# kogdenko/con-gen

Hardware: AMD Instinct MI355X
Metric: Gpkts/s + GB/s device-resident checksum, 64B & 1500B batches; %HBM peak (higher is better)
Workload: dtype u16; 1 GPU; 16777216 x 1500 B IPv4+TCP per GPU, dense stride 1500, ip_cksum + tcp_cksum per packet (BASELINE configs[2]; configs[4] at 8 GPUs); packets_per_gpu=16777216, packet_bytes=1500, parallelism=batch-split x1

## Files before the change

### con-gen_amd/csrc/cgck_dense_kernel.inc

```

constexpr int kDsS = 6;
constexpr uint32_t kDsSlot = kDsS * 1024;
constexpr int kDsChunks = kDsS * 64;
static_assert(((15 + 3 * 1520) >> 4) + 16 * (kDsS - 1) + 15 < kDsChunks, "a reducing lane's chunk lies in its slot");

template <int D, int C, bool W, int F>
__global__ __launch_bounds__(128) void CGCK_DSTR_KERNEL(KParams p)
{
	constexpr bool IP6 = CGCK_DSTR_IP6;
	static_assert(!IP6 || (W && F == 0), "the IPv6 variant is the product shape's: writer wave, no register frames");
	extern __shared__ __attribute__((aligned(16))) uint8_t smem[];
	const int lane = threadIdx.x & 63, g = lane >> 4, gl = lane & 15;
	const int wave = __builtin_amdgcn_readfirstlane(threadIdx.x >> 6);
	const uint32_t flags = p.flags;
	const bool raw = flags & CGCK_RAW;
	const int len = (int)p.ip_len;
	const uint32_t lds0 = __builtin_amdgcn_readfirstlane((uint32_t)(uintptr_t)smem);
	uint32_t *so = reinterpret_cast<uint32_t *>(smem + D * kDsSlot);
	const uint8_t *zero = (const uint8_t *)p.zero + (blockIdx.x & 63) * 64;
	const uint64_t base = reinterpret_cast<uint64_t>(p.base) + p.l3_off;
	const uint64_t n = p.n, stride = p.stride;
	constexpr uint32_t SC = 4 * C + F;
	const uint64_t NC = (n + SC - 1) / SC, G = gridDim.x, b = blockIdx.x;
	if (b >= NC)
		return;
	const uint32_t nsteps = (uint32_t)((NC - b + G - 1) / G * C);
	const uint32_t mode = p.contig;
	auto cfirst = [&](uint32_t k) { return (b + (uint64_t)k * G) * SC; };

	auto fin = [&](uint32_t tot, uint32_t ip, uint32_t ps, uint32_t hd, uint32_t proto) {
		const int hl = (int)hd * 4;
		uint32_t lo = 0, hi = 0;
		if (raw) {
			lo = finish(tot);
		} else if (len >= hl) {
			if (flags & CGCK_IP)
				lo = finish(ip);
			if (flags & CGCK_L4) {
				uint32_t L = ocsub(tot, ip);
				if (!(flags & CGCK_L4_NOPSEUDO))
					L = fold16(L + ps + (proto << 8) + bswap16((uint32_t)(len - hl) & 0xffffu));
				hi = finish(L);
			}
		}
		return lo | (hi << 16);
	};

	auto flush = [&](uint32_t k, const uint32_t *sb) {
		const uint64_t first = cfirst(k);
		if (first + 4 * C <= n) {
			if (lane < C) {
				const uint4 v4 = reinterpret_cast<const uint4 *>(sb)[lane];
				bstore16<kSc1>(out_rsrc(p.out + first, 16 * C), 16 * lane, u32x4_t{v4.x, v4.y, v4.z, v4.w});
			}
		} else {
			for (int i = lane; i < 4 * C; i += 64)
				if (first + i < n)
					gbl(p.out)[first + i] = sb[i];
		}
	};

	auto reg_frame = [&](uint64_t f, uint64_t a, int nch, const uint4 (&w)[kDsS]) __attribute__((always_inline)) {
		const int q = (int)(a & 15);
		uint32_t body = 0;
		uint4 tw = make_uint4(0, 0, 0, 0);
		bool ht = false;
#pragma unroll
		for (int s2 = 0; s2 < kDsS; ++s2) {
			const int c = 16 * s2 + gl;
			body += c < nch ? sum4(w[s2], 0u) : 0u;
			const bool t = c == nch - 1;
			const uint32_t mt = opaque(t ? ~0u : 0u);
			tw = make_uint4(pick(mt, w[s2].x, tw.x), pick(mt, w[s2].y, tw.y), pick(mt, w[s2].z, tw.z),
					pick(mt, w[s2].w, tw.w));
			ht = ht || t;
		}
		uint32_t corr = 0;
		if (gl == 0) {
			corr = hsum(q >= 4 ? w[0].x : 0u, 0);
			corr = hsum(q >= 8 ? w[0].y : 0u, corr);
			corr = hsum(q >= 12 ? w[0].z : 0u, corr);
		}
		if (ht) {
			const int e = q + len - 16 * (nch - 1);
			if ((len & 3) == 0) {
				corr = hsum(e <= 4 ? tw.y : 0u, corr);
				corr = hsum(e <= 8 ? tw.z : 0u, corr);
				corr = hsum(e <= 12 ? tw.w : 0u, corr);
			} else {
				corr = msum(tw, 0, e, 16, corr);
			}
		}
		uint32_t tot = fold16(body) + (0xffffu - fold16(corr));
		tot = fold16(gsum<16>(tot));
		const uint32_t n0 = __builtin_amdgcn_mov_dpp(w[0].x, 0x101, 0xF, 0xF, false);
		const uint32_t n1 = __builtin_amdgcn_mov_dpp(w[0].y, 0x101, 0xF, 0xF, false);
		const uint32_t n2 = __builtin_amdgcn_mov_dpp(w[0].z, 0x101, 0xF, 0xF, false);
		const uint32_t n3 = __builtin_amdgcn_mov_dpp(w[0].w, 0x101, 0xF, 0xF, false);
		const uint32_t d[8] = {w[0].x, w[0].y, w[0].z, w[0].w, n0, n1, n2, n3};
		const int q4 = q >> 2;
		const uint32_t m0 = opaque(q4 == 0 ? ~0u : 0u), m1 = opaque(q4 == 1 ? ~0u : 0u),
			       m2 = opaque(q4 == 2 ? ~0u : 0u);
		uint32_t h[5];
#pragma unroll
		for (int i = 0; i < 5; ++i)
			h[i] = pick(m0, d[i], pick(m1, d[i + 1], pick(m2, d[i + 2], d[i + 3])));
		const uint32_t hd = h[0] & 15;
		uint32_t ip = hsum(h[4], hsum(h[3], hsum(h[2], hsum(h[1], hsum(h[0], 0)))));
		if (gl == 0 && f < n) {
			if (hd != 5) {
				ip = 0;
				for (uint32_t i = 0; i < hd; ++i)
					ip = hsum(*gbl_at<const uint32_t>(a + 4 * i), ip);
			}
			const uint32_t r = fin(tot, fold16(ip), fold16(hsum(h[4], hsum(h[3], 0))), hd, (h[2] >> 8) & 0xffu);
			gbl(p.out)[f] = r;
			if (p.verdict)
				gbl(p.verdict)[f] = (uint8_t)(!raw && len < (int)hd * 4 ? CGCK_BAD_LEN : 0);
		}
	};

	if (W && wave == 1) {
		for (uint32_t j = 0; j < nsteps; ++j) {
			if (mode == 6)
				wg_barrier();
			if ((j + 1) % C == 0) {
				const uint32_t k = j / C;
				uint4 rw[F > 0 ? F / 4 : 1][kDsS];
				uint64_t ra[F > 0 ? F / 4 : 1];
				int rn[F > 0 ? F / 4 : 1];
#pragma unroll
				for (int u = 0; u < F / 4; ++u) {
					const uint64_t f = cfirst(k) + 4 * C + 4 * u + g;
					ra[u] = base + (f < n ? f : 0) * stride;
					rn[u] = f < n ? (int)(((ra[u] & 15) + len + 15) >> 4) : 0;
					const uint4 *c0 = reinterpret_cast<const uint4 *>(ra[u] & ~(uint64_t)15);
#pragma unroll
					for (int s2 = 0; s2 < kDsS; ++s2)
						rw[u][s2] = ldc<true>(c0, 16 * s2 + gl, rn[u], p.zero);
				}
				wg_barrier();
				const uint32_t *sb = so + (k & 1) * 8 * C;
				const uint64_t first = cfirst(k);
				for (int i = lane; i < 4 * C; i += 64) {
					const uint32_t v0 = sb[i], v1 = sb[4 * C + i];
					const uint32_t hd = (v1 >> 16) & 15u;
					if constexpr (IP6) {
						uint32_t bl = 0;
						const uint32_t r6 = first + i < n ? v6_dense(base + (first + i) * stride, len, v0 & 0xffffu,
											     v0 >> 16, v1 >> 24, flags, &bl)
										  : 0u;
						if (p.verdict && first + i < n)
							gbl(p.verdict)[first + i] = (uint8_t)bl;
						if (first + 4 * C <= n)
							bstore4<kSc1>(out_rsrc(p.out + first, 16 * C), 4 * i, r6);
						else if (first + i < n)
							gbl(p.out)[first + i] = r6;
						continue;
					}
					const uint32_t r = fin(v0 & 0xffffu, v0 >> 16, v1 & 0xffffu, hd, v1 >> 24);
					if (p.verdict && first + i < n)
						gbl(p.verdict)[first + i] = (uint8_t)(!raw && len < (int)hd * 4 ? CGCK_BAD_LEN : 0);
					if (first + 4 * C <= n)
						bstore4<kSc1>(out_rsrc(p.out + first, 16 * C), 4 * i, r);
					else if (first + i < n)
						gbl(p.out)[first + i] = r;
				}
#pragma unroll
				for (int u = 0; u < F / 4; ++u)
					reg_frame(cfirst(k) + 4 * C + 4 * u + g, ra[u], rn[u], rw[u]);
			}
		}
		return;
	}

	auto sfirst = [&](uint32_t j) { return cfirst(j / C) + 4 * (j % C); };
	auto issue = [&](uint32_t j) {
		const uint64_t f0 = sfirst(j);
		const bool live = j < nsteps && f0 < n;
		const uint64_t fl = f0 + 3 < n ? f0 + 3 : n - 1;
		const uint64_t a = (base + f0 * stride) & ~(uint64_t)15;
		const uint64_t e = (base + fl * stride + len - 1) & ~(uint64_t)15;
		const uint32_t slot = lds0 + (j % D) * kDsSlot;
#pragma unroll
		for (int i = 0; i < kDsS; ++i) {
			const uint64_t s0 = a + 1024 * i, src = s0 + 16 * lane;
			if (live && s0 + 1008 <= e)
				glds16_nt(reinterpret_cast<const void *>(src), slot + 1024 * i);
			else
				glds16_nt(live && src <= e ? reinterpret_cast<const void *>(src) : zero, slot + 1024 * i);
		}
	};
#pragma unroll
	for (int d = 0; d < D; ++d)
		issue(d);
	for (uint32_t j = 0; j < nsteps; ++j) {
		if (!W && j >= (uint32_t)C && (j % C) <= (uint32_t)(D - 1))
			asm volatile("s_waitcnt vmcnt(%0)" ::"i"(kDsS * (D - 1) + 1) : "memory");
		else
			asm volatile("s_waitcnt vmcnt(%0)" ::"i"(kDsS * (D - 1)) : "memory");
		if (!W || mode == 6)
			wg_barrier();
		uint32_t *sc = so + (W ? ((j / C) & 1) * 8 * C : 0);
		if (mode == 3) {
			issue(j + D);
		} else {
			const uint64_t f0 = sfirst(j);
			const uint64_t a = (base + f0 * stride) & ~(uint64_t)15;
			const int o = (int)(base + (f0 + g) * stride - a);
			const int q = o & 15, c0 = o >> 4;
			const int nch = (q + len + 15) >> 4;
			const uint8_t *sl = smem + (j % D) * kDsSlot;
			uint4 w[kDsS];
#pragma unroll
			for (int s = 0; s < kDsS; ++s) {
				const int c = c0 + 16 * s + gl;
				w[s] = *reinterpret_cast<const uint4 *>(sl + 16 * c);
			}
#if CGCK_DSTR_REGHDR
			asm volatile("s_waitcnt lgkmcnt(0)" ::: "memory");
			issue(j + D);
			uint4 wt = make_uint4(0, 0, 0, 0);
			bool ht = false;
#pragma unroll
			for (int s = 0; s < kDsS; ++s) {
				const bool t = 16 * s + gl == nch - 1;
				const uint32_t mt = opaque(t ? ~0u : 0u);
				wt = make_uint4(pick(mt, w[s].x, wt.x), pick(mt, w[s].y, wt.y), pick(mt, w[s].z, wt.z),
						pick(mt, w[s].w, wt.w));
				ht = ht || t;
			}
			const uint32_t n0 = __builtin_amdgcn_mov_dpp(w[0].x, 0x101, 0xF, 0xF, false);
			const uint32_t n1 = __builtin_amdgcn_mov_dpp(w[0].y, 0x101, 0xF, 0xF, false);
			const uint32_t n2 = __builtin_amdgcn_mov_dpp(w[0].z, 0x101, 0xF, 0xF, false);
			const uint32_t n3 = __builtin_amdgcn_mov_dpp(w[0].w, 0x101, 0xF, 0xF, false);
			const uint32_t dd[8] = {w[0].x, w[0].y, w[0].z, w[0].w, n0, n1, n2, n3};
			const int q4 = q >> 2;
			const uint32_t m0 = opaque(q4 == 0 ? ~0u : 0u), m1 = opaque(q4 == 1 ? ~0u : 0u),
				       m2 = opaque(q4 == 2 ? ~0u : 0u);
			uint32_t hh[5];
#pragma unroll
			for (int i = 0; i < 5; ++i)
				hh[i] = pick(m0, dd[i], pick(m1, dd[i + 1], pick(m2, dd[i + 2], dd[i + 3])));
			const uint32_t h1 = hh[1], h2 = hh[2], h3 = hh[3], h4 = hh[4];
			const uint32_t hd = hh[0] & 15;
			uint32_t ip = IP6 ? hsum(h1, hsum(hh[0], 0)) : hsum(h4, hsum(h3, hsum(h2, hsum(h1, hsum(hh[0], 0)))));
			if (!IP6 && gl == 0 && hd != 5 && f0 + g < n) {
				const uint64_t fa = base + (f0 + g) * stride;
				ip = 0;
				for (uint32_t i = 0; i < hd; ++i)
					ip = hsum(*gbl_at<const uint32_t>(fa + 4 * i), ip);
			}
#else
			const uint4 wt = *reinterpret_cast<const uint4 *>(sl + 16 * (c0 + nch - 1));
			const uint32_t *hw = reinterpret_cast<const uint32_t *>(sl + o);
			const uint32_t h0 = hw[0], h1 = hw[1], h2 = hw[2], h3 = hw[3], h4 = hw[4];
			const uint32_t hd = h0 & 15;
			uint32_t ip = IP6 ? hsum(h1, hsum(h0, 0)) : hsum(h4, hsum(h3, hsum(h2, hsum(h1, hsum(h0, 0)))));
			if (!IP6 && hd != 5) {
				ip = 0;
				for (uint32_t i = 0; i < hd; ++i)
					ip = hsum(hw[i], ip);
			}
			asm volatile("s_waitcnt lgkmcnt(0)" ::: "memory");
			issue(j + D);
#endif

			uint32_t cs[kDsS];
#pragma unroll
			for (int s = 0; s < kDsS; ++s)
				cs[s] = sum4(w[s], 0);
			uint32_t body = 0;
#pragma unroll
			for (int s = 0; s < kDsS; ++s)
				body += (len >= 1280 && s < 5) || 16 * s + gl < nch ? cs[s] : 0u;
			uint32_t lead = hsum(q >= 4 ? w[0].x : 0u, 0);
			lead = hsum(q >= 8 ? w[0].y : 0u, lead);
			lead = hsum(q >= 12 ? w[0].z : 0u, lead);
			const int e = q + len - 16 * (nch - 1);
			uint32_t tail;
			if ((len & 3) == 0) {
				tail = hsum(e <= 4 ? wt.y : 0u, 0);
				tail = hsum(e <= 8 ? wt.z : 0u, tail);
				tail = hsum(e <= 12 ? wt.w : 0u, tail);
			} else {
				tail = msum(wt, 0, e, 16, 0);
			}
#if CGCK_DSTR_REGHDR
			const uint32_t corr = (gl == 0 ? lead : 0u) + (ht ? tail : 0u);
#else
			const uint32_t corr = gl == 0 ? lead + tail : 0u;
#endif
			uint32_t tot = fold16(body) + (0xffffu - fold16(corr));
			tot = fold16(gsum<16>(tot));

			const uint32_t proto = IP6 ? (h1 >> 16) & 0xffu : (h2 >> 8) & 0xffu;
			const uint32_t ps = fold16(hsum(h4, hsum(h3, 0)));
			if (W) {
				if (gl == 0) {
					sc[4 * (j % C) + g] = tot | (fold16(ip) << 16);
					sc[4 * C + 4 * (j % C) + g] = ps | (hd << 16) | (proto << 24);
				}
			} else if (gl == 0) {
				sc[4 * (j % C) + g] = fin(tot, fold16(ip), ps, hd, proto);
			}
		}
		if ((j + 1) % C == 0) {
			asm volatile("s_waitcnt lgkmcnt(0)" ::: "memory");
			if (W)
				wg_barrier();
			else if (mode != 2)
				flush(j / C, sc);
		}
	}
	asm volatile("s_waitcnt vmcnt(0)" ::: "memory");
}
```

### con-gen_amd/csrc/cgck_device.h

```cpp
#pragma once
#include <hip/hip_runtime.h>
#include <stdint.h>

#include "cgck_internal.h"

namespace cgck {

#define CGCK_GLOBAL __attribute__((address_space(1)))

__device__ __forceinline__ uint32_t hsum(uint32_t w, uint32_t acc)
{
	typedef unsigned short us2 __attribute__((ext_vector_type(2)));
	us2 a = __builtin_bit_cast(us2, w);
	us2 one = {1, 1};
	return __builtin_amdgcn_udot2(a, one, acc, false);
}

__device__ __forceinline__ uint32_t sum4(const uint4 &w, uint32_t acc)
{
	return hsum(w.w, hsum(w.z, hsum(w.y, hsum(w.x, acc))));
}

__device__ __forceinline__ uint32_t bmask(int s, int e)
{
	uint32_t hm = e >= 4 ? 0xffffffffu : ((1u << (8 * e)) - 1u);
	uint32_t lm = 0xffffffffu << (8 * (s & 3));
	return e > s ? (hm & lm) : 0u;
}

__device__ __forceinline__ int clamp4(int x)
{
	return min(max(x, 0), 4);
}

__device__ __forceinline__ uint32_t dmask(int co, int i, int r0, int r1)
{
	int b = co + 4 * i;
	return bmask(clamp4(r0 - b), clamp4(r1 - b));
}

__device__ __forceinline__ uint32_t msum(const uint4 &w, int co, int r0, int r1, uint32_t acc)
{
	acc = hsum(w.x & dmask(co, 0, r0, r1), acc);
	acc = hsum(w.y & dmask(co, 1, r0, r1), acc);
	acc = hsum(w.z & dmask(co, 2, r0, r1), acc);
	acc = hsum(w.w & dmask(co, 3, r0, r1), acc);
	return acc;
}

__device__ __forceinline__ void zero_bytes(uint4 &w, int co, int r0, int r1)
{
	w.x &= ~dmask(co, 0, r0, r1);
	w.y &= ~dmask(co, 1, r0, r1);
	w.z &= ~dmask(co, 2, r0, r1);
	w.w &= ~dmask(co, 3, r0, r1);
}

__device__ __forceinline__ uint32_t cmask16(int co, int r0, int r1)
{
	const int s = min(max(r0 - co, 0), 16), e = min(max(r1 - co, 0), 16);
	return e > s ? ((1u << e) - 1u) & ~((1u << s) - 1u) : 0u;
}

__device__ __forceinline__ uint32_t nibmask(uint32_t m, int i)
{
	const uint32_t n = (m >> (4 * i)) & 15u;
	return ((n * 0x00204081u) & 0x01010101u) * 0xffu;
}

__device__ __forceinline__ uint32_t msum16(const uint4 &w, uint32_t m, uint32_t acc)
{
	acc = hsum(w.x & nibmask(m, 0), acc);
	acc = hsum(w.y & nibmask(m, 1), acc);
	acc = hsum(w.z & nibmask(m, 2), acc);
	acc = hsum(w.w & nibmask(m, 3), acc);
	return acc;
}

__device__ __forceinline__ void zero16(uint4 &w, uint32_t m)
{
	w.x &= ~nibmask(m, 0);
	w.y &= ~nibmask(m, 1);
	w.z &= ~nibmask(m, 2);
	w.w &= ~nibmask(m, 3);
}

template <int G>
__device__ __forceinline__ uint32_t gsum(uint32_t v)
{
	v += __builtin_amdgcn_mov_dpp(v, 0xB1, 0xF, 0xF, false);
	v += __builtin_amdgcn_mov_dpp(v, 0x4E, 0xF, 0xF, false);
	if (G >= 8)
		v += __builtin_amdgcn_mov_dpp(v, 0x141, 0xF, 0xF, false);
	if (G >= 16)
		v += __builtin_amdgcn_mov_dpp(v, 0x140, 0xF, 0xF, false);
	if (G >= 32)
		v += __shfl_xor(v, 16, 64);
	if (G >= 64)
		v += __shfl_xor(v, 32, 64);
	return v;
}

__device__ __forceinline__ uint32_t fold16(uint32_t x)
{
	x = (x & 0xffffu) + (x >> 16);
	x = (x & 0xffffu) + (x >> 16);
	x = (x & 0xffffu) + (x >> 16);
	return x;
}

__device__ __forceinline__ uint32_t bswap16(uint32_t x)
{
	return ((x & 0xffu) << 8) | ((x >> 8) & 0xffu);
}

__device__ __forceinline__ uint32_t finish(uint32_t f)
{
	uint32_t r = (~f) & 0xffffu;
	return r ? r : 0xffffu;
}

__device__ __forceinline__ bool l4_nopseudo(uint32_t proto, uint32_t flags)
{
	return (flags & CGCK_L4_NOPSEUDO) || ((flags & kFlagL4Auto) && proto == 1);
}

__device__ __forceinline__ int l4_field(uint32_t proto, uint32_t flags)
{
	if (l4_nopseudo(proto, flags))
		return proto == 1 ? 2 : -1;
	return proto == 6 ? 16 : (proto == 17 ? 6 : -1);
}

__device__ __forceinline__ uint32_t rx_meta(uint32_t avail, uint32_t b0, uint32_t tl_hi, uint32_t tl_lo,
					    uint32_t proto, uint32_t *cover)
{
	const uint32_t hl = (b0 & 15) * 4;
	if (avail < 20 || hl < 20 || hl > avail) {
		*cover = 0;
		return 0;
	}
	const uint32_t total = tl_hi << 8 | tl_lo;
	uint32_t cv = total < avail ? total : avail;
	*cover = cv < hl ? hl : cv;
	const uint32_t l4len = total >= hl ? total - hl : 0;
	const uint32_t need = proto == 6 ? 18 : proto == 17 ? 8 : proto == 1 ? 4 : 0xffffffffu;
	uint32_t m = kRxOkIp | (proto == 1 ? kRxIcmp : 0) | hl << 8 | l4len << 16;
	if (total >= hl && total <= avail && l4len >= need)
		m |= kRxOkL4;
	return m;
}

__device__ __forceinline__ void store16(uint8_t *p, uint32_t v)
{
	if ((reinterpret_cast<uintptr_t>(p) & 1) == 0) {
		*(CGCK_GLOBAL uint16_t *)p = (uint16_t)v;
	} else {
		((CGCK_GLOBAL uint8_t *)p)[0] = (uint8_t)v;
		((CGCK_GLOBAL uint8_t *)p)[1] = (uint8_t)(v >> 8);
	}
}

template <bool SYS>
__device__ __forceinline__ void st32p(CGCK_GLOBAL uint32_t *p, uint32_t v)
{
	if (SYS)
		__hip_atomic_store(p, v, __ATOMIC_RELAXED, __HIP_MEMORY_SCOPE_SYSTEM);
	else
		*p = v;
}

template <bool SYS>
__device__ __forceinline__ void st8p(CGCK_GLOBAL uint8_t *p, uint8_t v)
{
	if (SYS)
		__hip_atomic_store(p, v, __ATOMIC_RELAXED, __HIP_MEMORY_SCOPE_SYSTEM);
	else
		*p = v;
}

template <bool SYS>
__device__ __forceinline__ void store16p(uint8_t *p, uint32_t v)
{
	if (!SYS) {
		store16(p, v);
	} else if ((reinterpret_cast<uintptr_t>(p) & 1) == 0) {
		__hip_atomic_store((CGCK_GLOBAL uint16_t *)p, (uint16_t)v, __ATOMIC_RELAXED, __HIP_MEMORY_SCOPE_SYSTEM);
	} else {
		__hip_atomic_store((CGCK_GLOBAL uint8_t *)p, (uint8_t)v, __ATOMIC_RELAXED, __HIP_MEMORY_SCOPE_SYSTEM);
		__hip_atomic_store((CGCK_GLOBAL uint8_t *)p + 1, (uint8_t)(v >> 8), __ATOMIC_RELAXED,
				   __HIP_MEMORY_SCOPE_SYSTEM);
	}
}

typedef unsigned int u32x4_t __attribute__((ext_vector_type(4)));

template <class T>
__device__ __forceinline__ CGCK_GLOBAL T *gbl(T *p)
{
	return (CGCK_GLOBAL T *)p;
}

template <class T>
__device__ __forceinline__ CGCK_GLOBAL T *gbl_at(uint64_t a)
{
	return (CGCK_GLOBAL T *)a;
}

__device__ __forceinline__ void glds16_nt(const void *gsrc, uint32_t lds_dst)
{
	uint32_t keep;
	asm volatile("s_mov_b32 %0, m0\n\ts_mov_b32 m0, %2\n\ts_nop 0\n\tglobal_load_lds_dwordx4 %1, off nt\n\t"
		     "s_mov_b32 m0, %0"
		     : "=&s"(keep)
		     : "v"(gsrc), "s"(lds_dst)
		     : "memory");
}

constexpr int kSc1 = 16, kNt = 2, kDefaultPolicy = 0;
__device__ __forceinline__ __amdgpu_buffer_rsrc_t out_rsrc(const void *base, uint32_t bytes)
{
	return __builtin_amdgcn_make_buffer_rsrc(const_cast<void *>(base), 0, (int)bytes, 0x00020000);
}
template <int POLICY>
__device__ __forceinline__ void bstore16(__amdgpu_buffer_rsrc_t r, uint32_t off, u32x4_t v)
{
	__builtin_amdgcn_raw_buffer_store_b128(v, r, (int)off, 0, POLICY);
}
template <int POLICY>
__device__ __forceinline__ void bstore4(__amdgpu_buffer_rsrc_t r, uint32_t off, uint32_t v)
{
	__builtin_amdgcn_raw_buffer_store_b32(v, r, (int)off, 0, POLICY);
}

__device__ __forceinline__ void wg_barrier()
{
	asm volatile("s_barrier" ::: "memory");
}

#ifndef CGCK_FLUSH_POLICY
#define CGCK_FLUSH_POLICY 0
#endif
__device__ __forceinline__ void flush_u32(const uint32_t *src, uint32_t *dst, int count, int t, int nt)
{
#if CGCK_FLUSH_POLICY == 0
	for (int i = t; i < count; i += nt)
		__builtin_nontemporal_store(src[i], (CGCK_GLOBAL uint32_t *)dst + i);
#elif CGCK_FLUSH_POLICY == 1
	for (int i = t; i < count; i += nt)
		asm volatile("global_store_dword %0, %1, off sc1" ::"v"(dst + i), "v"(src[i]) : "memory");
#else
	int head = (int)(((16 - ((uintptr_t)dst & 15)) & 15) >> 2);
	head = head < count ? head : count;
	if (t < head)
		asm volatile("global_store_dword %0, %1, off sc1" ::"v"(dst + t), "v"(src[t]) : "memory");
	const int body = (count - head) >> 2;
	for (int i = t; i < body; i += nt) {
		const uint32_t *s4 = src + head + 4 * i;
		const u32x4_t v = {s4[0], s4[1], s4[2], s4[3]};
#if CGCK_FLUSH_POLICY == 3
		asm volatile("global_store_dwordx4 %0, %1, off nt\n\ts_nop 1" ::"v"(dst + head + 4 * i), "v"(v) : "memory");
#else
		asm volatile("global_store_dwordx4 %0, %1, off sc1\n\ts_nop 1" ::"v"(dst + head + 4 * i), "v"(v) : "memory");
#endif
	}
	for (int i = head + 4 * body + t; i < count; i += nt)
		asm volatile("global_store_dword %0, %1, off sc1" ::"v"(dst + i), "v"(src[i]) : "memory");
#endif
}

template <bool NT>
__device__ __forceinline__ uint4 ld(const uint4 *p)
{
	if (NT) {
		u32x4_t x = __builtin_nontemporal_load((const CGCK_GLOBAL u32x4_t *)p);
		return make_uint4(x[0], x[1], x[2], x[3]);
	}
	const u32x4_t x = *(const CGCK_GLOBAL u32x4_t *)p;
	return make_uint4(x[0], x[1], x[2], x[3]);
}

template <bool NT>
__device__ __forceinline__ uint4 ldc(const uint4 *c0, int i, int nch, const void *zero)
{
	return ld<NT>(nch > 0 ? c0 + min(i, nch - 1) : reinterpret_cast<const uint4 *>(zero));
}

template <int N>
__device__ __forceinline__ void ld_sys16xN(const uint4 *const (&a)[N], uint4 (&v)[N]);

__device__ __forceinline__ void ld_sys16x2(const uint4 *p0, const uint4 *p1, uint4 &v0, uint4 &v1)
{
	u32x4_t a, b;
	asm volatile("global_load_dwordx4 %0, %2, off sc0 sc1\n\t"
		     "global_load_dwordx4 %1, %3, off sc0 sc1\n\t"
		     "s_waitcnt vmcnt(0)"
		     : "=&v"(a), "=&v"(b)
		     : "v"(p0), "v"(p1)
		     : "memory");
	v0 = make_uint4(a[0], a[1], a[2], a[3]);
	v1 = make_uint4(b[0], b[1], b[2], b[3]);
}

template <>
__device__ __forceinline__ void ld_sys16xN<2>(const uint4 *const (&a)[2], uint4 (&v)[2])
{
	ld_sys16x2(a[0], a[1], v[0], v[1]);
}

template <>
__device__ __forceinline__ void ld_sys16xN<6>(const uint4 *const (&a)[6], uint4 (&v)[6])
{
	u32x4_t r0, r1, r2, r3, r4, r5;
	asm volatile("global_load_dwordx4 %0, %6, off sc0 sc1\n\t"
		     "global_load_dwordx4 %1, %7, off sc0 sc1\n\t"
		     "global_load_dwordx4 %2, %8, off sc0 sc1\n\t"
		     "global_load_dwordx4 %3, %9, off sc0 sc1\n\t"
		     "global_load_dwordx4 %4, %10, off sc0 sc1\n\t"
		     "global_load_dwordx4 %5, %11, off sc0 sc1\n\t"
		     "s_waitcnt vmcnt(0)"
		     : "=&v"(r0), "=&v"(r1), "=&v"(r2), "=&v"(r3), "=&v"(r4), "=&v"(r5)
		     : "v"(a[0]), "v"(a[1]), "v"(a[2]), "v"(a[3]), "v"(a[4]), "v"(a[5])
		     : "memory");
	v[0] = make_uint4(r0[0], r0[1], r0[2], r0[3]);
	v[1] = make_uint4(r1[0], r1[1], r1[2], r1[3]);
	v[2] = make_uint4(r2[0], r2[1], r2[2], r2[3]);
	v[3] = make_uint4(r3[0], r3[1], r3[2], r3[3]);
	v[4] = make_uint4(r4[0], r4[1], r4[2], r4[3]);
	v[5] = make_uint4(r5[0], r5[1], r5[2], r5[3]);
}

template <bool NT>
struct GChunks {
	const uint4 *p;
	__device__ __forceinline__ uint4 operator[](int i) const { return ld<NT>(p + i); }
};

struct Sched {
	uint64_t it, end, step;
};

__device__ __forceinline__ Sched sched(uint64_t n_iters, bool contig, uint32_t bid, uint32_t nb)
{
	Sched s;
	if (contig) {
		const uint64_t per = (n_iters + nb - 1) / nb;
		s.it = (uint64_t)bid * per;
		s.end = s.it + per < n_iters ? s.it + per : n_iters;
		s.step = 1;
	} else {
		s.it = bid;
		s.end = n_iters;
		s.step = nb;
	}
	return s;
}

__device__ __forceinline__ Sched sched(uint64_t n_iters, bool contig)
{
	return sched(n_iters, contig, blockIdx.x, gridDim.x);
}

struct Pkt {
	uint64_t a0;
	uint32_t len;
	bool ok;
};

template <bool DESC>
__device__ __forceinline__ Pkt get_pkt(const KParams &p, uint64_t k)
{
	Pkt r;
	r.ok = k < p.n;
	uint64_t kk = r.ok ? k : 0;
	if (DESC) {
		const CGCK_GLOBAL uint32_t *d = (const CGCK_GLOBAL uint32_t *)p.desc + 3 * kk;
		uint32_t lo = d[0], hi = d[1], w2 = d[2];
		uint64_t fo = ((uint64_t)hi << 32) | lo;
		r.a0 = reinterpret_cast<uint64_t>(p.base) + fo + (w2 & 0xffffu);
		r.len = w2 >> 16;
	} else {
		r.a0 = reinterpret_cast<uint64_t>(p.base) + kk * p.stride + p.l3_off;
		r.len = p.ip_len;
	}
	if (!r.ok)
		r.len = 0;
	return r;
}

typedef __attribute__((address_space(3))) const uint32_t lds_u32;
typedef __attribute__((address_space(3))) const u32x4_t lds_v4;
typedef __attribute__((address_space(3))) const uint8_t lds_u8;

template <bool NT, bool LDSP>
__device__ __forceinline__ uint4 ldq(const uint4 *p)
{
	if constexpr (LDSP) {
		const u32x4_t v = *(lds_v4 *)p;
		return make_uint4(v[0], v[1], v[2], v[3]);
	} else {
		return ld<NT>(p);
	}
}

template <bool NT, bool LDSP>
__device__ __forceinline__ uint4 ldcq(const uint4 *c0, int i, int nch, const void *zero)
{
	return ldq<NT, LDSP>(nch > 0 ? c0 + min(i, nch - 1) : reinterpret_cast<const uint4 *>(zero));
}

template <bool LDSP>
__device__ __forceinline__ uint32_t ld8q(uint64_t a)
{
	return LDSP ? (uint32_t) * (lds_u8 *)(const uint8_t *)a : (uint32_t)*gbl_at<const uint8_t>(a);
}
__device__ __forceinline__ Pkt get_pkt_lds(const KParams &p, uint64_t k)
{
	Pkt r;
	r.ok = k < p.n;
	const uint32_t kk = r.ok ? (uint32_t)k : 0u;
	lds_u32 *d = (lds_u32 *)(const uint32_t *)p.desc + 3 * kk;
	const uint32_t lo = d[0], hi = d[1], w2 = d[2];
	r.a0 = reinterpret_cast<uint64_t>(p.base) + (((uint64_t)hi << 32) | lo) + (w2 & 0xffffu);
	r.len = r.ok ? w2 >> 16 : 0u;
	return r;
}

__device__ __forceinline__ bool desc_inside(uint32_t lo, uint32_t hi, uint32_t w2, uint64_t limit)
{
	const uint64_t fo = ((uint64_t)hi << 32) | lo;
	return fo <= limit && (w2 & 0xffffu) + (w2 >> 16) <= limit - fo;
}

__device__ __forceinline__ uint32_t pick(uint32_t m, uint32_t a, uint32_t b)
{
	return (a & m) | (b & ~m);
}

__device__ __forceinline__ uint32_t opaque(uint32_t m)
{
	asm volatile("" : "+v"(m));
	return m;
}

__device__ __forceinline__ uint32_t ocsub(uint32_t x, uint32_t y)
{
	return fold16(x + (0xffffu - y));
}


struct Part {
	uint32_t tot, ip, ps, fld;
};

template <bool HDR>
__device__ __forceinline__ void eat(Part &pt, uint4 w, int k, int q, int len, int hl, int fo,
				    uint32_t flags)
{
	const int co = k * 16;
	if (HDR && co < q + 80) {
		if (flags & (CGCK_VERIFY | CGCK_ZERO_FIELDS)) {
			const uint32_t mf = cmask16(co, q + 10, q + 12);
			const uint32_t mg = fo >= 0 ? cmask16(co, q + hl + fo, q + hl + fo + 2) : 0u;
			const uint32_t f = msum16(w, mf, 0);
			const uint32_t g = msum16(w, mg, 0);
			pt.fld += f | (g << 16);
			zero16(w, mf | mg);
		}
		pt.ip = msum16(w, cmask16(co, q, q + hl), pt.ip);
		pt.ps = msum16(w, cmask16(co, q + 12, q + 20), pt.ps);
	}
	if (co >= q && co + 16 <= q + len)
		pt.tot = sum4(w, pt.tot);
	else
		pt.tot = msum16(w, cmask16(co, q, q + len), pt.tot);
}


constexpr int kV6Ok = 0, kV6NoL4 = 1, kV6BadLen = 2;
constexpr int kV6MaxExt = 8;

__host__ __device__ __forceinline__ bool v6_is_ext(uint32_t nh)
{
	return nh == 0 || nh == 43 || nh == 60 || nh == 51;
}

__host__ __device__ __forceinline__ int v6_field(uint32_t nh)
{
	return nh == 6 ? 16 : nh == 17 ? 6 : nh == 58 ? 2 : -1;
}

struct V6 {
	int l4_off;
	uint32_t nh;
	int st;
};

__device__ __forceinline__ V6 v6_walk(uint64_t a0, int len, uint32_t nh0)
{
	V6 r = {40, nh0, kV6Ok};
	if (len < 40) {
		r.st = kV6BadLen;
		return r;
	}
	for (int i = 0;; ++i) {
		if (r.l4_off > len) {
			r.st = kV6BadLen;
			return r;
		}
		if (r.nh == 44) {
			r.st = kV6NoL4;
			return r;
		}
		if (!v6_is_ext(r.nh))
			break;
		if (i == kV6MaxExt || r.l4_off + 2 > len) {
			r.st = kV6BadLen;
			return r;
		}
		const uint32_t next = *gbl_at<const uint8_t>(a0 + r.l4_off);
		const uint32_t hl = *gbl_at<const uint8_t>(a0 + r.l4_off + 1);
		r.l4_off += r.nh == 51 ? (int)(hl + 2) * 4 : (int)(hl + 1) * 8;
		r.nh = next;
	}
	const int fo = v6_field(r.nh);
	if (fo >= 0 && r.l4_off + fo + 2 > len)
		r.st = kV6BadLen;
	return r;
}

__device__ __forceinline__ uint32_t v6_dense(uint64_t a0, int len, uint32_t tot, uint32_t h8, uint32_t nh0,
					     uint32_t flags, uint32_t *verdict)
{
	*verdict = 0;
	if (len < 40) {
		*verdict = CGCK_BAD_LEN;
		return 0;
	}
	if (!(flags & CGCK_L4))
		return 0;
	const V6 v = v6_walk(a0, len, nh0);
	if (v.st == kV6BadLen)
		*verdict = CGCK_BAD_LEN;
	if (v.st != kV6Ok)
		return 0;
	uint32_t ext = 0;
	for (int o = 40; o < v.l4_off; o += 4)
		ext = hsum(*gbl_at<const uint32_t>(a0 + o), ext);
	uint32_t L = ocsub(ocsub(tot, h8), fold16(ext));
	L = fold16(L + (v.nh << 8) + bswap16((uint32_t)(len - v.l4_off) & 0xffffu));
	return finish(L) << 16;
}

template <bool HDR>
__device__ __forceinline__ void eat6(Part &pt, uint4 w, int k, int q, int len, int l4, int fa, uint32_t flags)
{
	const int co = k * 16;
	if ((flags & (CGCK_VERIFY | CGCK_ZERO_FIELDS)) && fa >= 0) {
		const uint32_t mg = cmask16(co, q + fa, q + fa + 2);
		pt.fld += msum16(w, mg, 0) << 16;
		zero16(w, mg);
	}
	if (HDR && co < q + 48)
		pt.ps = msum16(w, cmask16(co, q + 8, q + 40), pt.ps);
	if (co >= q + l4 && co + 16 <= q + len)
		pt.tot = sum4(w, pt.tot);
	else
		pt.tot = msum16(w, cmask16(co, q + l4, q + len), pt.tot);
}

}
```

Before: 4.411 Gpkt/s.

## Hoist per-step address math and specialize LDS-load issue on whole-KiB count

Moves per-packet offset, mask and chunk-count computation out of the step loop, since the stride is uniform and every step has the same intra-slot layout. Folds the tail, lead and body selection into masked udot2 multipliers. Replaces the generic per-chunk global-to-LDS issue with inline-asm sequences specialized at compile time on the number of full KiB chunks, advancing M0 and a running address instead of recomputing bounds. A generic tail loop handles the final partial steps. This cuts scalar and vector instruction overhead in the hot loop, at the cost of more template instantiations and fragile hand-written asm that manages M0.

```diff
diff --git a/con-gen_amd/csrc/cgck_dense_kernel.inc b/con-gen_amd/csrc/cgck_dense_kernel.inc
--- a/con-gen_amd/csrc/cgck_dense_kernel.inc
+++ b/con-gen_amd/csrc/cgck_dense_kernel.inc
@@ -3,6 +3,43 @@
 constexpr uint32_t kDsSlot = kDsS * 1024;
 constexpr int kDsChunks = kDsS * 64;
 static_assert(((15 + 3 * 1520) >> 4) + 16 * (kDsS - 1) + 15 < kDsChunks, "a reducing lane's chunk lies in its slot");
+
+#define CGCK_DS_OPEN "s_mov_b32 %[k], m0\n\ts_mov_b32 m0, %[slot]\n\ts_nop 2\n\t"
+#define CGCK_DS_NEXT "s_add_u32 m0, m0, 0x400\n\ts_nop 0\n\t"
+#define CGCK_DS_W(i) "global_load_lds_dwordx4 %[o" #i "], %[a] nt\n\t" CGCK_DS_NEXT
+#define CGCK_DS_P "global_load_lds_dwordx4 %[pa], off nt\n\t"
+#define CGCK_DS_Z CGCK_DS_NEXT "global_load_lds_dwordx4 %[vz], %[z] nt\n\t"
+#define CGCK_DS_ASM(body)                                                                               \
+	asm volatile(CGCK_DS_OPEN body "s_mov_b32 m0, %[k]"                                              \
+		     : [k] "=&s"(keep)                                                                   \
+		     : [slot] "s"(slot), [a] "s"(a), [o0] "v"(off[0]), [o1] "v"(off[1]), [o2] "v"(off[2]), \
+		       [o3] "v"(off[3]), [o4] "v"(off[4]), [pa] "v"(pa), [vz] "v"(vz), [z] "s"(z)        \
+		     : "memory", "scc")
+template <int NW>
+__device__ __forceinline__ void dstr_issue_full(uint64_t a, uint32_t slot, const uint32_t (&off)[kDsS - 1], const void *pa,
+						 const void *z, uint32_t vz)
+{
+	static_assert(NW >= 0 && NW < kDsS, "a step of four frames (<= 6091 bytes) has at most five whole KiBs");
+	uint32_t keep;
+	if constexpr (NW == 5)
+		CGCK_DS_ASM(CGCK_DS_W(0) CGCK_DS_W(1) CGCK_DS_W(2) CGCK_DS_W(3) CGCK_DS_W(4) CGCK_DS_P);
+	else if constexpr (NW == 4)
+		CGCK_DS_ASM(CGCK_DS_W(0) CGCK_DS_W(1) CGCK_DS_W(2) CGCK_DS_W(3) CGCK_DS_P CGCK_DS_Z);
+	else if constexpr (NW == 3)
+		CGCK_DS_ASM(CGCK_DS_W(0) CGCK_DS_W(1) CGCK_DS_W(2) CGCK_DS_P CGCK_DS_Z CGCK_DS_Z);
+	else if constexpr (NW == 2)
+		CGCK_DS_ASM(CGCK_DS_W(0) CGCK_DS_W(1) CGCK_DS_P CGCK_DS_Z CGCK_DS_Z CGCK_DS_Z);
+	else if constexpr (NW == 1)
+		CGCK_DS_ASM(CGCK_DS_W(0) CGCK_DS_P CGCK_DS_Z CGCK_DS_Z CGCK_DS_Z CGCK_DS_Z);
+	else
+		CGCK_DS_ASM(CGCK_DS_P CGCK_DS_Z CGCK_DS_Z CGCK_DS_Z CGCK_DS_Z CGCK_DS_Z);
+}
+#undef CGCK_DS_ASM
+#undef CGCK_DS_Z
+#undef CGCK_DS_P
+#undef CGCK_DS_W
+#undef CGCK_DS_NEXT
+#undef CGCK_DS_OPEN
 
 template <int D, int C, bool W, int F>
 __global__ __launch_bounds__(128) void CGCK_DSTR_KERNEL(KParams p)
@@ -25,7 +62,11 @@
 	if (b >= NC)
 		return;
 	const uint32_t nsteps = (uint32_t)((NC - b + G - 1) / G * C);
+#if CGCK_LAB
 	const uint32_t mode = p.contig;
+#else
+	constexpr uint32_t mode = 0;
+#endif
 	auto cfirst = [&](uint32_t k) { return (b + (uint64_t)k * G) * SC; };
 
 	auto fin = [&](uint32_t tot, uint32_t ip, uint32_t ps, uint32_t hd, uint32_t proto) {
@@ -191,10 +232,51 @@
 				glds16_nt(live && src <= e ? reinterpret_cast<const void *>(src) : zero, slot + 1024 * i);
 		}
 	};
+	static_assert(SC % 4 == 0, "a step's first frame is a multiple of 4");
+	static_assert(D < C, "the prologue's steps lie in the first chunk");
+	const int al = (int)(base & 15);
+	const int o = al + g * (int)stride;
+	const int q = o & 15, c0 = o >> 4;
+	const int nch = (q + len + 15) >> 4;
+	const int e = q + len - 16 * (nch - 1);
+	const uint32_t rd_w = opaque(16u * (uint32_t)(c0 + gl));
+	[[maybe_unused]] const uint32_t rd_t = opaque(16u * (uint32_t)(c0 + nch - 1));
+	[[maybe_unused]] const uint32_t rd_h = opaque((uint32_t)o);
+	uint32_t bmul[kDsS];
+#pragma unroll
+	for (int s = 0; s < kDsS; ++s)
+		bmul[s] = opaque(16 * s + gl < nch ? kHsumAll : 0u);
+	const uint32_t lm1 = opaque(gl == 0 && q >= 4 ? kHsumAll : 0u), lm2 = opaque(gl == 0 && q >= 8 ? kHsumAll : 0u),
+		       lm3 = opaque(gl == 0 && q >= 12 ? kHsumAll : 0u);
+#if CGCK_DSTR_REGHDR
+	const bool tl = true;
+#else
+	const bool tl = gl == 0;
+#endif
+	const uint32_t tm0 = opaque(tl ? dmask(0, 0, e, 16) : 0u), tm1 = opaque(tl ? dmask(0, 1, e, 16) : 0u),
+		       tm2 = opaque(tl ? dmask(0, 2, e, 16) : 0u), tm3 = opaque(tl ? dmask(0, 3, e, 16) : 0u);
+
+	const uint32_t span = ((uint32_t)al + 3 * (uint32_t)stride + (uint32_t)len - 1) & ~15u;
+	const uint32_t nw = (span + 16) >> 10;
+	uint32_t off[kDsS - 1];
+#pragma unroll
+	for (int i = 0; i < kDsS - 1; ++i)
+		off[i] = opaque(1024u * i + 16u * lane);
+	const uint32_t poff = 1024 * nw + 16 * lane;
+	const uint32_t pmask = opaque(poff <= span ? ~0u : 0u);
+	const uint32_t vz = opaque(0u);
+	const uint32_t klast = nsteps / C - 1;
+	const uint64_t lrem = (n - cfirst(klast)) / 4;
+	const uint32_t jfull = klast * C + (lrem < (uint64_t)C ? (uint32_t)lrem : (uint32_t)C);
+	const uint64_t step4 = 4 * stride, cjump = (G * SC - 4 * (C - 1)) * stride;
+	uint64_t ia = base - (uint64_t)al + (cfirst(0) + 4 * D) * stride;
+	uint32_t slot_off = 0;
+
 #pragma unroll
 	for (int d = 0; d < D; ++d)
 		issue(d);
-	for (uint32_t j = 0; j < nsteps; ++j) {
+	auto step = [&](uint32_t j, auto nwc) __attribute__((always_inline)) {
+		constexpr int NW = decltype(nwc)::value;
 		if (!W && j >= (uint32_t)C && (j % C) <= (uint32_t)(D - 1))
 			asm volatile("s_waitcnt vmcnt(%0)" ::"i"(kDsS * (D - 1) + 1) : "memory");
 		else
@@ -202,24 +284,32 @@
 		if (!W || mode == 6)
 			wg_barrier();
 		uint32_t *sc = so + (W ? ((j / C) & 1) * 8 * C : 0);
+		auto refill = [&]() __attribute__((always_inline)) {
+			if constexpr (NW >= 0) {
+				const uint32_t slot = lds0 + slot_off;
+				const uint64_t pl = ia + poff;
+				const uint64_t zl = reinterpret_cast<uint64_t>(zero);
+				const void *pa = reinterpret_cast<const void *>(
+					(uint64_t)pick(pmask, (uint32_t)pl, (uint32_t)zl) |
+					(uint64_t)pick(pmask, (uint32_t)(pl >> 32), (uint32_t)(zl >> 32)) << 32);
+				dstr_issue_full<NW>(ia, slot, off, pa, zero, vz);
+				ia += ((j + D + 1) % C) == 0 ? cjump : step4;
+			} else {
+				issue(j + D);
+			}
+		};
 		if (mode == 3) {
-			issue(j + D);
+			refill();
 		} else {
-			const uint64_t f0 = sfirst(j);
-			const uint64_t a = (base + f0 * stride) & ~(uint64_t)15;
-			const int o = (int)(base + (f0 + g) * stride - a);
-			const int q = o & 15, c0 = o >> 4;
-			const int nch = (q + len + 15) >> 4;
-			const uint8_t *sl = smem + (j % D) * kDsSlot;
+			const uint8_t *sl = smem + slot_off;
 			uint4 w[kDsS];
 #pragma unroll
-			for (int s = 0; s < kDsS; ++s) {
-				const int c = c0 + 16 * s + gl;
-				w[s] = *reinterpret_cast<const uint4 *>(sl + 16 * c);
-			}
+			for (int s = 0; s < kDsS; ++s)
+				w[s] = *reinterpret_cast<const uint4 *>(sl + rd_w + 256 * s);
 #if CGCK_DSTR_REGHDR
 			asm volatile("s_waitcnt lgkmcnt(0)" ::: "memory");
-			issue(j + D);
+			refill();
+			const uint64_t f0 = sfirst(j);
 			uint4 wt = make_uint4(0, 0, 0, 0);
 			bool ht = false;
 #pragma unroll
@@ -252,8 +342,8 @@
 					ip = hsum(*gbl_at<const uint32_t>(fa + 4 * i), ip);
 			}
 #else
-			const uint4 wt = *reinterpret_cast<const uint4 *>(sl + 16 * (c0 + nch - 1));
-			const uint32_t *hw = reinterpret_cast<const uint32_t *>(sl + o);
+			const uint4 wt = *reinterpret_cast<const uint4 *>(sl + rd_t);
+			const uint32_t *hw = reinterpret_cast<const uint32_t *>(sl + rd_h);
 			const uint32_t h0 = hw[0], h1 = hw[1], h2 = hw[2], h3 = hw[3], h4 = hw[4];
 			const uint32_t hd = h0 & 15;
 			uint32_t ip = IP6 ? hsum(h1, hsum(h0, 0)) : hsum(h4, hsum(h3, hsum(h2, hsum(h1, hsum(h0, 0)))));
@@ -263,34 +353,25 @@
 					ip = hsum(hw[i], ip);
 			}
 			asm volatile("s_waitcnt lgkmcnt(0)" ::: "memory");
-			issue(j + D);
+			refill();
 #endif
 
 			uint32_t cs[kDsS];
 #pragma unroll
 			for (int s = 0; s < kDsS; ++s)
-				cs[s] = sum4(w[s], 0);
+				cs[s] = sum4_sel(w[s], bmul[s], 0);
 			uint32_t body = 0;
 #pragma unroll
 			for (int s = 0; s < kDsS; ++s)
-				body += (len >= 1280 && s < 5) || 16 * s + gl < nch ? cs[s] : 0u;
-			uint32_t lead = hsum(q >= 4 ? w[0].x : 0u, 0);
-			lead = hsum(q >= 8 ? w[0].y : 0u, lead);
-			lead = hsum(q >= 12 ? w[0].z : 0u, lead);
-			const int e = q + len - 16 * (nch - 1);
-			uint32_t tail;
-			if ((len & 3) == 0) {
-				tail = hsum(e <= 4 ? wt.y : 0u, 0);
-				tail = hsum(e <= 8 ? wt.z : 0u, tail);
-				tail = hsum(e <= 12 ? wt.w : 0u, tail);
-			} else {
-				tail = msum(wt, 0, e, 16, 0);
-			}
+				body += cs[s];
+			const uint32_t lead = hsum_sel(w[0].z, lm3, hsum_sel(w[0].y, lm2, hsum_sel(w[0].x, lm1, 0)));
 #if CGCK_DSTR_REGHDR
-			const uint32_t corr = (gl == 0 ? lead : 0u) + (ht ? tail : 0u);
+			const uint32_t tsel = ht ? ~0u : 0u;
 #else
-			const uint32_t corr = gl == 0 ? lead + tail : 0u;
+			constexpr uint32_t tsel = ~0u;
 #endif
+			const uint32_t tail = hsum(wt.w & tm3 & tsel, hsum(wt.z & tm2 & tsel, hsum(wt.y & tm1 & tsel, hsum(wt.x & tm0 & tsel, 0))));
+			const uint32_t corr = lead + tail;
 			uint32_t tot = fold16(body) + (0xffffu - fold16(corr));
 			tot = fold16(gsum<16>(tot));
 
@@ -305,6 +386,7 @@
 				sc[4 * (j % C) + g] = fin(tot, fold16(ip), ps, hd, proto);
 			}
 		}
+		slot_off = slot_off + kDsSlot == D * kDsSlot ? 0 : slot_off + kDsSlot;
 		if ((j + 1) % C == 0) {
 			asm volatile("s_waitcnt lgkmcnt(0)" ::: "memory");
 			if (W)
@@ -312,6 +394,22 @@
 			else if (mode != 2)
 				flush(j / C, sc);
 		}
+	};
+	const uint32_t jhot = (jfull > (uint32_t)D ? jfull : (uint32_t)D) - D;
+	uint32_t j = 0;
+	auto hot = [&](auto nwc) __attribute__((always_inline)) {
+		for (; j < jhot; ++j)
+			step(j, nwc);
+	};
+	switch (nw) {
+	case 5: hot(std::integral_constant<int, 5>{}); break;
+	case 4: hot(std::integral_constant<int, 4>{}); break;
+	case 3: hot(std::integral_constant<int, 3>{}); break;
+	case 2: hot(std::integral_constant<int, 2>{}); break;
+	case 1: hot(std::integral_constant<int, 1>{}); break;
+	default: hot(std::integral_constant<int, 0>{}); break;
 	}
+	for (; j < nsteps; ++j)
+		step(j, std::integral_constant<int, -1>{});
 	asm volatile("s_waitcnt vmcnt(0)" ::: "memory");
 }
diff --git a/con-gen_amd/csrc/cgck_device.h b/con-gen_amd/csrc/cgck_device.h
--- a/con-gen_amd/csrc/cgck_device.h
+++ b/con-gen_amd/csrc/cgck_device.h
@@ -19,6 +19,18 @@
 __device__ __forceinline__ uint32_t sum4(const uint4 &w, uint32_t acc)
 {
 	return hsum(w.w, hsum(w.z, hsum(w.y, hsum(w.x, acc))));
+}
+
+constexpr uint32_t kHsumAll = 0x00010001u;
+__device__ __forceinline__ uint32_t hsum_sel(uint32_t w, uint32_t mul, uint32_t acc)
+{
+	typedef unsigned short us2 __attribute__((ext_vector_type(2)));
+	return __builtin_amdgcn_udot2(__builtin_bit_cast(us2, w), __builtin_bit_cast(us2, mul), acc, false);
+}
+
+__device__ __forceinline__ uint32_t sum4_sel(const uint4 &w, uint32_t mul, uint32_t acc)
+{
+	return hsum_sel(w.w, mul, hsum_sel(w.z, mul, hsum_sel(w.y, mul, hsum_sel(w.x, mul, acc))));
 }
 
 __device__ __forceinline__ uint32_t bmask(int s, int e)
```

Result: faster. 4.542 Gpkt/s, median of 6 (+3.0%).
